# Duankaiwen/LSNet

Measured on AMD Instinct MI355X. Metric: img/s train LSNet R-50-FPN 1333x800 bs2/GPU, higher is better.
Workload: dtype f32 (fp32-equivalent: 6 bf16 MFMA terms per product on exact 3-way operand splits, fp32 accumulate); 1 GPU; LSNet R50-FPN bbox (conv_module_type=dcn), 2 img/GPU 3x800x1344 (1333x800 padded to /32), 7 gt/img, fwd+bwd+gradient arena (the reducer's buckets, no collective on one rank)+clip35+SGD; global_batch=2, parallelism=dp1, world_size=1, memory_format=channels_last, launch=eager

## Files before the change

### lsnet_amd/csrc/conv.hip

```cpp
#include <hip/hip_runtime.h>
#include <stdint.h>
#include <string.h>

#include <type_traits>
#include <vector>

#include "conv_kernels.h"
#include "conv_wgrad_kernels.h"
#include "lib_state.h"
#include "prof.h"

namespace lsn {

static int conv_np() { return math_np() == 0 ? 6 : math_np(); }
static int conv_npl() { return split_npl(conv_np()); }

struct RJob {
    bool fold;
    const float *part, *part_b;
    float *gw, *gb;
    size_t n;
    int nb, splits, splits_b, R, Co;
    WgFold f;
};
// ... 308 lines not shown
struct BwdClass {
    TapSub ts;
    int py, px, pad_h, pad_w, dstep;
    size_t wf_off;
};
struct BwdPlan {
    BwdClass cls[64];
    int ncls;
    bool need_zero;
    size_t bytes;
};

static int bwd_plan(int C, int Co, int kh, int kw, int s, int pad, int dil, BwdPlan *pl)
{
    if (s * s > 64) return fail(LSN_ERR_UNSUPPORTED, "conv2d backward-data: stride %d is not supported", s);
    pl->ncls = 0, pl->need_zero = false, pl->bytes = 0;
    auto taps_of = [&](int p, int k, int &t0, int &tstep, int &nt) {
        t0 = -1, tstep = 1, nt = 0;
        int prev = -1;
        for (int t = 0; t < k; ++t)
            if (((p + pad - t * dil) % s + s) % s == 0) {
                if (nt == 0) t0 = t;
                if (nt == 1) tstep = t - prev;
                prev = t;
                ++nt;
            }
    };
    for (int py = 0; py < s; ++py)
        for (int px = 0; px < s; ++px) {
            BwdClass c;
            c.py = py, c.px = px;
            taps_of(py, kh, c.ts.i0, c.ts.istep, c.ts.ni);
            taps_of(px, kw, c.ts.j0, c.ts.jstep, c.ts.nj);
            c.ts.kw = kw;
            if (c.ts.ni == 0 || c.ts.nj == 0) {
                pl->need_zero = true;
                continue;
            }
            const int dstep_h = c.ts.istep * dil / s, dstep_w = c.ts.jstep * dil / s;
            if (c.ts.ni > 1 && c.ts.nj > 1 && dstep_h != dstep_w)
                return fail(LSN_ERR_UNSUPPORTED, "conv2d backward-data: unequal tap spacing");
            c.dstep = c.ts.ni > 1 ? dstep_h : (c.ts.nj > 1 ? dstep_w : 1);
            if ((c.ts.ni > 1 && c.ts.istep * dil % s != 0) || (c.ts.nj > 1 && c.ts.jstep * dil % s != 0))
                return fail(LSN_ERR_UNSUPPORTED, "conv2d backward-data: stride / dilation combination");
            const int q0h = (py + pad - c.ts.i0 * dil) / s, q0w = (px + pad - c.ts.j0 * dil) / s;
            c.pad_h = (c.ts.ni - 1) * c.dstep - q0h;
            c.pad_w = (c.ts.nj - 1) * c.dstep - q0w;
            c.wf_off = pl->bytes;
            pl->bytes += cv_wfrag_bytes(C, c.ts.ni * c.ts.nj, Co, conv_npl());
            pl->cls[pl->ncls++] = c;
        }
    return 0;
}

static int conv_backward_data_impl(int n, const lsn_conv_level *lv, const void *prepared, int C, int Co, int kh, int kw,
                                   int stride, int pad, int dil, hipStream_t st)
{
    LSN_CHECK(n >= 1 && n <= CV_MAXLV && lv && prepared, "conv2d backward: bad arguments");
    LaunchLog log(1, n, lv, C, C, Co, kh, kw, stride, pad, dil, 0, st);
    if (Co % 4 != 0 && C <= 64) return fail(LSN_ERR_UNSUPPORTED, "conv2d backward-data: Co %% 4 != 0 needs C > 64");
    const int s = stride;
    int Ho[CV_MAXLV], Wo[CV_MAXLV];
    for (int i = 0; i < n; ++i) {
        LSN_CHECK(lv[i].x && lv[i].out, "conv2d backward: NULL tensor in level %d", i);
        if (int rc = conv_check(lv[i].B, lv[i].H, lv[i].W, C, Co, kh, kw, stride, pad, dil, &Ho[i], &Wo[i])) return rc;
    }
    if (s > 1 && n > 1) return fail(LSN_ERR_UNSUPPORTED, "conv2d backward-data: strided convolutions take one level per call");
    BwdPlan pl;
    if (int rc = bwd_plan(C, Co, kh, kw, s, pad, dil, &pl)) return rc;
    const int H = lv[0].H, W = lv[0].W, B = lv[0].B;
    bool epi = false;
    for (int i = 0; i < n; ++i) epi = epi || lv[i].residual || lv[i].gate;
    if (epi && pl.need_zero)
        return fail(LSN_ERR_UNSUPPORTED, "conv2d backward-data: residual / gate with residue classes that have no tap");
    if (epi && C % 4 != 0) return fail(LSN_ERR_UNSUPPORTED, "conv2d backward-data: residual / gate need C %% 4 == 0");
    if (pl.need_zero) LSN_HIP(hipMemsetAsync(lv[0].out, 0, sizeof(float) * (size_t)B * H * W * C, st));
    for (int ci = 0; ci < pl.ncls; ++ci) {
        const BwdClass &c = pl.cls[ci];
        const int Hc = c.py < H ? (H - c.py + s - 1) / s : 0, Wc = c.px < W ? (W - c.px + s - 1) / s : 0;
        if (s > 1 && (Hc == 0 || Wc == 0)) continue;
        ConvArgs a = {};
        a.wf = reinterpret_cast<const unsigned short *>(reinterpret_cast<const unsigned char *>(prepared) + c.wf_off);
        a.wf_bytes = (int)cv_wfrag_bytes(C, c.ts.ni * c.ts.nj, Co, conv_npl());
        a.nlv = n;
        for (int i = 0; i < n; ++i) {
            ConvLvl &L = a.lv[i];
            L.x = lv[i].x, L.out = lv[i].out, L.res = lv[i].residual, L.gate = lv[i].gate;
            L.B = lv[i].B, L.H = Ho[i], L.W = Wo[i];
            L.Ho = s > 1 ? Hc : lv[i].H, L.Wo = s > 1 ? Wc : lv[i].W;
            L.P = L.B * L.Ho * L.Wo;
        }
        a.C = Co, a.Co = C, a.kh = c.ts.ni, a.kw = c.ts.nj, a.stride = 1;
        a.xpitch = Co;
        a.pad_h = c.pad_h, a.pad_w = c.pad_w, a.dil = c.dstep;
        if (s > 1) a.ostep = s, a.oy0 = c.py, a.ox0 = c.px, a.OH = H, a.OW = W;
        ConvProf prof(PROF_CONV_BWD_DATA, a, st);
        if (int rc = conv_forward(a, st)) return rc;
    }
    return 0;
}

static int64_t prepared_bytes(int kind, int C, int Co, int kh, int kw, int stride, int pad, int dil)
{
    if (kind == 0) return (int64_t)cv_wfrag_bytes(Co, kh * kw, C, conv_npl());
    if (kind == 2) return (int64_t)cv_wfrag_bytes(kh * kw * C, 1, Co, conv_npl());
    BwdPlan pl;
    if (bwd_plan(C, Co, kh, kw, stride, pad, dil, &pl)) return -1;
    return (int64_t)pl.bytes;
}

static int bn_fold_of(const lsn_conv_wprep &p, BnFold *bn)
{
    *bn = BnFold();
    if (!p.bn_gamma) return 0;
    LSN_CHECK(p.bn_var, "conv2d prepare: incomplete BatchNorm description");
    if (p.kind == 0)
        LSN_CHECK(p.bn_beta && p.bn_mean && p.shift_out, "conv2d prepare: incomplete BatchNorm description");
    else
        LSN_CHECK(!p.shift_out, "conv2d prepare: the shift belongs to the forward image");
    bn->gamma = p.bn_gamma, bn->var = p.bn_var, bn->beta = p.bn_beta, bn->mean = p.bn_mean, bn->shift_out = p.shift_out;
    bn->eps = p.bn_eps;
    return 0;
}

static int prepare_weights(int kind, const float *w, void *prepared, int C, int Co, int kh, int kw, int stride, int pad,
                           int dil, hipStream_t st, const BnFold &bn = BnFold())
{
    LSN_CHECK(w && prepared, "conv2d prepare: NULL pointer");
    LSN_CHECK(C > 0 && Co > 0 && kh > 0 && kw > 0, "conv2d prepare: bad weight shape");
    if (kh * kw > 64) return fail(LSN_ERR_UNSUPPORTED, "conv2d kernel takes at most 64 taps, got %d x %d", kh, kw);
    if (prepared_bytes(kind, C, Co, kh, kw, stride, pad, dil) >= ((int64_t)1 << 31))
        return fail(LSN_ERR_UNSUPPORTED, "conv2d: weight too large for 32-bit buffer offsets");
    if (kind == 0) {
        if (int rc = conv_wfrag(w, reinterpret_cast<unsigned short *>(prepared), Co, kh * kw, C, 0, TapSub{}, st, bn)) return rc;
    } else if (kind == 2) {
        if (int rc = conv_wfrag(w, reinterpret_cast<unsigned short *>(prepared), kh * kw * C, 1, Co, 1, TapSub{0, 1, 1, 0, 1, 1, 1}, st,
                                bn))
            return rc;
    } else {
        BwdPlan pl;
        if (int rc = bwd_plan(C, Co, kh, kw, stride, pad, dil, &pl)) return rc;
        for (int ci = 0; ci < pl.ncls; ++ci)
            if (int rc = conv_wfrag(w, reinterpret_cast<unsigned short *>(reinterpret_cast<unsigned char *>(prepared) + pl.cls[ci].wf_off),
                                    C, kh * kw, Co, 1, pl.cls[ci].ts, st, bn))
                return rc;
    }
    LSN_HIP(hipGetLastError());
    return 0;
}

static thread_local const WgFoldJobs *g_wg_fold = nullptr;
bool conv_wgrad_fold_pending() { return g_wg_fold != nullptr; }
static int wg_jobs() { return g_wg_fold ? g_wg_fold->njobs : 1; }
template <int TI, int TJ, int TG, int WI, int WJ, int PMAX, bool UN_OK>
static int launch_wgrad_cfg(WgArgs &a, float *gw, float *gb, int accumulate, hipStream_t st)
{
    const bool un = a.Co % 4 != 0;
    if (un && !UN_OK) return 1;
    constexpr int BN = WI * TI * 32, BM = WJ * TJ * 32;
    const int npl = conv_npl(), K = a.kh * a.kw;
    const int blocks = cdiv(a.Co, BM) * cdiv(a.C, BN);
    const size_t nW = (size_t)a.Co * K * a.C;
    const int nj = wg_jobs();
    int S = 512 / (blocks * nj);
    const size_t cap = ((size_t)192 << 20) / 4 / (nW + a.Co) / nj;
    if ((size_t)S > cap) S = (int)cap;
    if (S > a.nseg / nj / 6) S = a.nseg / nj / 6;
    if (S < 1) S = 1;
    S *= nj;
    float *part = nullptr;
    if (int rc = wgrad_part_buffer((size_t)S * (nW + a.Co) + 16, &part, st)) return rc;
    a.part = part;
    a.part_b = part + (((size_t)S * nW + 3) & ~(size_t)3);
    a.want_bias = gb != nullptr;
    constexpr int XP = 1024 / BN, GP = 1024 / BM;
    const size_t lds = (size_t)2 * npl * ((size_t)cdiv(PMAX, XP) * XP * BN * 2 + (size_t)cdiv(16, GP) * GP * BM * 2);
    if (lds > 160 * 1024) return 1;
    dim3 grid(blocks, S);
    LSN_CHECK((long long)a.nseg * (S + 1) < (1ll << 32), "conv2d backward-weight: %d segments x %d splits exceed the kernel's 32-bit split arithmetic", a.nseg, S);
    auto launch = [&](auto kern) -> int {
        LSN_HIP(hipFuncSetAttribute(reinterpret_cast<const void *>(kern), hipFuncAttributeMaxDynamicSharedMemorySize, (int)lds));
        hipLaunchKernelGGL(kern, grid, dim3(256), lds, st, a);
        return 0;
    };
    int rc;
    constexpr bool FINE = !(TG == 9 && WI == 4);
    rc = split_dispatch(conv_np(), [&](auto np) {
        constexpr int NP = decltype(np)::value;
        if constexpr (NP == 1 && TG == 9 && WI == 4) {
            return fail(LSN_ERR_INVALID, "conv2d backward-weight: no one-product form of the narrow 3x3 kernel");
        } else {
            if constexpr (UN_OK) {
                if (un) return launch(conv_wgrad_kernel<TI, TJ, TG, WI, WJ, NP, true, PMAX, false>);
            }
            return launch(conv_wgrad_kernel<TI, TJ, TG, WI, WJ, NP, false, PMAX, FINE>);
        }
    });
    if (rc) return rc;
    return conv_wgrad_reduce(a.part, gw, nW, a.part_b, gb, a.Co, S, S, accumulate, st);
}

static int reduce_ls(int splits)
{
    constexpr int PER_LANE = 16;
    int LS = 1;
    while (LS < 64 && LS * PER_LANE <= splits) LS <<= 1;
    return LS;
}

int conv_wgrad_reduce(const float *part, float *gw, size_t n, const float *part_b, float *gb, int nb, int splits, int splits_b,
                      int accumulate, hipStream_t st)
{
    const int nj = wg_jobs();
    if (g_wg_fold)
        LSN_CHECK(part_b && nb > 0 && n % ((size_t)nb * 4) == 0 && splits % nj == 0 && splits_b % nj == 0,
                  "conv2d backward-weight (folded norm): bad partial layout");
    if (Arena *ar = accumulate ? deferring(st) : nullptr) {
        bool clash = false;
        for (const RJob &q : *ar->jobs)
            for (int j = 0; j < nj; ++j) {
                const float *tw = g_wg_fold ? (nj > 1 ? g_wg_fold->gw[j] : gw) : gw;
                clash = clash || q.gw == tw || (gb && q.gb == gb) || (g_wg_fold && q.fold && q.f.dgamma == g_wg_fold->f[j].dgamma);
            }
        if (clash)
            if (int rc = wgrad_flush(ar)) return rc;
        for (int j = 0; j < nj; ++j) {
            RJob q = {};
            q.fold = g_wg_fold != nullptr;
            q.part = part + (size_t)j * (splits / nj) * n, q.part_b = q.fold ? part_b + (size_t)j * (splits_b / nj) * nb : part_b;
            q.gw = nj > 1 ? g_wg_fold->gw[j] : gw, q.gb = q.fold ? nullptr : gb;
            q.n = n, q.nb = nb, q.splits = splits / nj, q.splits_b = splits_b / nj;
            if (q.fold) q.R = (int)(n / nb), q.Co = nb, q.f = g_wg_fold->f[j];
            ar->jobs->push_back(q);
        }
        if ((long long)(ar->used * sizeof(float)) > (ar->defer_mb << 20)) {
            if (int rc = wgrad_flush(ar)) return rc;
            ar->used = 0;
        }
        return 0;
    }
    const int LS = reduce_ls(splits / nj);
    if (g_wg_fold) {
        hipLaunchKernelGGL(conv_wgrad_reduce_bn_kernel, dim3(nb, nj), dim3(256), 0, st, part, gw, (int)(n / nb), nb, part_b,
                           splits / nj, splits_b / nj, accumulate, LS, *g_wg_fold);
        LSN_HIP(hipGetLastError());
        return 0;
    }
    const size_t thr = n / 4 * LS;
    const int rb = (int)((thr + 255) / 256 < 4096 ? (thr + 255) / 256 : 4096);
    hipLaunchKernelGGL(conv_wgrad_reduce_kernel, dim3(rb > 0 ? rb : 1), dim3(256), 0, st, part, gw, n, part_b, gb, nb, splits,
                       splits_b, accumulate, LS);
    LSN_HIP(hipGetLastError());
    return 0;
}

static int wgrad_flush(Arena *ar)
{
    std::vector<RJob> &jobs = *ar->jobs;
    if (jobs.empty()) return 0;
    hipStream_t st = ar->st;
    double bytes = 0;
    for (const RJob &q : jobs) bytes += 4.0 * ((double)q.splits * q.n + 2.0 * q.n);
    ProfSpan prof(PROF_CONV_WGRAD, 0.0, bytes, st);
    RJobsPlain P = {};
    RJobsFold F = {};
    int pblk = 0, fblk = 0;
    auto launch_plain = [&]() {
        if (P.njobs) hipLaunchKernelGGL(conv_wgrad_reduce_multi_kernel, dim3(pblk), dim3(256), 0, st, P);
        P.njobs = 0, pblk = 0;
    };
    auto launch_fold = [&]() {
        if (F.njobs) hipLaunchKernelGGL(conv_wgrad_reduce_bn_multi_kernel, dim3(fblk), dim3(256), 0, st, F);
        F.njobs = 0, fblk = 0;
    };
    for (const RJob &q : jobs) {
        const int LS = reduce_ls(q.splits);
        if (q.fold) {
            if (F.njobs == RJ_MAX) launch_fold();
            RJobFold &d = F.j[F.njobs++];
            d.part = q.part, d.part_b = q.part_b, d.gw = q.gw, d.f = q.f, d.R = q.R, d.Co = q.Co, d.splits = q.splits,
            d.splits_b = q.splits_b, d.LS = LS, d.blk0 = fblk;
            fblk += q.Co;
        } else {
            if (P.njobs == RJ_MAX) launch_plain();
            const size_t thr = q.n / 4 * LS;
            const int rb = (int)((thr + 255) / 256 < 4096 ? (thr + 255) / 256 : 4096);
            RJobPlain &d = P.j[P.njobs++];
            d.part = q.part, d.part_b = q.part_b, d.gw = q.gw, d.gb = q.gb, d.n = q.n, d.nb = q.nb, d.splits = q.splits,
            d.splits_b = q.splits_b, d.LS = LS, d.blk0 = pblk, d.nblk = rb > 0 ? rb : 1;
            pblk += d.nblk;
        }
    }
    launch_plain();
    launch_fold();
    jobs.clear();
    LSN_HIP(hipGetLastError());
    return 0;
}

int conv_wgrad_mm(int n, const lsn_conv_level *lv, float *gw, float *gb, int C, int Co, int kh, int kw, int stride, int pad,
                  int dil, int accumulate, hipStream_t st)
{
    const bool k33 = kh == 3 && kw == 3 && stride == 1 && dil == 1, k11 = kh == 1 && kw == 1;
    if (n < 1 || n > CV_MAXLV || !(k33 || k11) || C % 4 != 0) return 1;
    WgArgs a = {};
    int seg = 0;
    for (int i = 0; i < n; ++i) {
        WgLvl &L = a.lv[i];
        const int B = lv[i].B, H = lv[i].H, W = lv[i].W;
        if (!lv[i].x || !lv[i].grad_out || B <= 0 || H <= 0 || W <= 0) return 1;
        const int Ho = conv_out_size(H, kh, stride, pad, dil), Wo = conv_out_size(W, kw, stride, pad, dil);
        if (Ho <= 0 || Wo <= 0) return 1;
        if ((int64_t)B * H * W * C * 4 >= ((int64_t)1 << 31) || (int64_t)B * Ho * Wo * Co * 4 >= ((int64_t)1 << 31)) return 1;
        L.x = lv[i].x, L.go = lv[i].grad_out, L.B = B, L.H = H, L.W = W, L.Ho = Ho, L.Wo = Wo;
        L.nsx = cdiv(Wo, 16);
        L.seg0 = seg;
        seg += B * Ho * L.nsx;
    }
    a.nlv = n, a.nseg = seg;
    a.C = C, a.Co = Co, a.kh = kh, a.kw = kw, a.stride = stride, a.pad = pad, a.dil = dil;
    a.cstep = kw == 1 ? stride : 1;
    a.PW = kw == 1 ? 16 : 15 * stride + (kw - 1) * dil + 1;
    if (kh * a.PW > 99) return 1;
    if (kh * kw == 9 && Co <= 32 && conv_np() == 1) return 1;
    double px = 0, in_el = 0;
    for (int i = 0; i < n; ++i) px += (double)a.lv[i].B * a.lv[i].Ho * a.lv[i].Wo, in_el += (double)a.lv[i].B * a.lv[i].H * a.lv[i].W * C;
    ProfSpan prof(PROF_CONV_WGRAD, 2.0 * px * Co * C * kh * kw, 4.0 * (in_el + px * Co + (double)Co * kh * kw * C), st);
    if (kh * kw == 1) {
        if (C <= 64)
            return Co <= 64 ? launch_wgrad_cfg<1, 1, 1, 2, 2, 16, false>(a, gw, gb, accumulate, st)
                            : launch_wgrad_cfg<1, 2, 1, 2, 2, 16, false>(a, gw, gb, accumulate, st);
        return Co <= 64 ? launch_wgrad_cfg<2, 1, 1, 2, 2, 16, false>(a, gw, gb, accumulate, st)
                        : launch_wgrad_cfg<2, 2, 1, 2, 2, 16, false>(a, gw, gb, accumulate, st);
    }
    if (Co <= 32) return launch_wgrad_cfg<1, 1, 9, 4, 1, 54, true>(a, gw, gb, accumulate, st);
    return launch_wgrad_cfg<1, 1, 9, 2, 2, 54, false>(a, gw, gb, accumulate, st);
}

static WfragJob *g_jobs_dev = nullptr;
static size_t g_jobs_cap = 0;
static std::vector<WfragJob> g_jobs_host;

static int prepare_weights_multi(int n, const lsn_conv_wprep *it, hipStream_t st)
{
    LSN_CHECK(n >= 0 && (n == 0 || it), "conv2d prepare: bad item list");
    std::vector<WfragJob> jobs;
    long long total = 0;
    for (int i = 0; i < n; ++i) {
        const lsn_conv_wprep &p = it[i];
        LSN_CHECK(p.w && p.prepared && p.C > 0 && p.Co > 0 && p.kh > 0 && p.kw > 0 && p.kh * p.kw <= 64,
                  "conv2d prepare: bad item %d", i);
        if (prepared_bytes(p.kind, p.C, p.Co, p.kh, p.kw, p.stride, p.pad, p.dil) >= ((int64_t)1 << 31))
            return fail(LSN_ERR_UNSUPPORTED, "conv2d: weight too large for 32-bit buffer offsets");
        BnFold bn;
        if (int rc = bn_fold_of(p, &bn)) return rc;
        auto add = [&](void *out, int Co, int K, int C, int flipT, const TapSub &ts) {
            WfragJob j;
            wfrag_job(j, p.w, reinterpret_cast<unsigned short *>(out), Co, K, C, flipT, ts, bn);
            j.start = total;
            total += wfrag_threads(j);
            jobs.push_back(j);
        };
        if (p.kind == 0) {
            add(p.prepared, p.Co, p.kh * p.kw, p.C, 0, TapSub{});
        } else if (p.kind == 2) {
            add(p.prepared, p.kh * p.kw * p.C, 1, p.Co, 1, TapSub{0, 1, 1, 0, 1, 1, 1});
        } else {
            BwdPlan pl;
            if (int rc = bwd_plan(p.C, p.Co, p.kh, p.kw, p.stride, p.pad, p.dil, &pl)) return rc;
            for (int c = 0; c < pl.ncls; ++c)
                add(reinterpret_cast<unsigned char *>(p.prepared) + pl.cls[c].wf_off, p.C, p.kh * p.kw, p.Co, 1, pl.cls[c].ts);
        }
    }
    if (jobs.empty()) return 0;
    const size_t bytes = jobs.size() * sizeof(WfragJob);
    const bool same = jobs.size() == g_jobs_host.size() && memcmp(jobs.data(), g_jobs_host.data(), bytes) == 0;
    if (!same) {
        if (jobs.size() > g_jobs_cap) {
            LSN_HIP(hipMalloc(reinterpret_cast<void **>(&g_jobs_dev), (jobs.size() + 64) * sizeof(WfragJob)));
            lib_stat(STAT_MALLOCS, 1), lib_stat(STAT_HELD_BYTES, (long long)((jobs.size() + 64) * sizeof(WfragJob)));
            g_jobs_cap = jobs.size() + 64;
        }
        LSN_HIP(hipStreamSynchronize(st));
        lib_stat(STAT_BLOCKING_SYNCS, 1);
        LSN_HIP(hipMemcpy(g_jobs_dev, jobs.data(), bytes, hipMemcpyHostToDevice));
        g_jobs_host = jobs;
    }
    const int blocks = (int)((total + 255) / 256 < 4096 ? (total + 255) / 256 : 4096);
    if (int rc = split_dispatch(conv_np(), [&](auto np) {
            hipLaunchKernelGGL(conv_wfrag_multi_kernel<SplitCfg<decltype(np)::value>::NPL>, dim3(blocks), dim3(256), 0, st, g_jobs_dev,
                               (int)jobs.size(), total);
            return 0;
        }))
        return rc;
    LSN_HIP(hipGetLastError());
    return 0;
}

}

extern "C" {

int lsn_wgrad_defer(int max_mbytes, lsn_stream_t stream)
{
    hipStream_t st = reinterpret_cast<hipStream_t>(stream);
    lsn::Arena *ar = lsn::arena_of(st);
    if (max_mbytes > 0) {
        if (int rc = lsn::arena_get(st, &ar)) return rc;
        if (!ar->jobs) ar->jobs = new std::vector<lsn::RJob>();
        ar->jobs->clear();
        ar->used = 0;
        ar->defer_mb = max_mbytes;
        return 0;
    }
    if (!ar) return 0;
    const int rc = lsn::wgrad_flush(ar);
    ar->defer_mb = 0, ar->used = 0;
    return rc;
}

int lsn_wgrad_flush(lsn_stream_t stream)
{
    lsn::Arena *ar = lsn::arena_of(reinterpret_cast<hipStream_t>(stream));
    if (!ar) return 0;
    const int rc = lsn::wgrad_flush(ar);
    ar->used = 0;
    return rc;
}

int lsn_conv2d_backward_weight_bn(const float *x, const float *g, const float *w, const float *bn_gamma, const float *bn_mean,
                                  const float *bn_var, float bn_eps, float *grad_w, float *grad_gamma, float *grad_beta, int B,
                                  int H, int W, int C, int Co, int kh, int kw, int stride, int pad, int dil, int accumulate,
                                  lsn_stream_t stream)
{
    LSN_CHECK(x && g && w && bn_gamma && bn_mean && bn_var && grad_w && grad_gamma && grad_beta,
              "conv2d backward-weight (folded norm): NULL pointer");
    if (((size_t)kh * kw * C) % 4 != 0)
        return lsn::fail(LSN_ERR_UNSUPPORTED, "conv2d backward-weight (folded norm): kh * kw * C %% 4 != 0");
    lsn::WgFoldJobs f = {};
    f.f[0] = lsn::WgFold{w, bn_gamma, bn_mean, bn_var, grad_gamma, grad_beta, bn_eps};
    f.gw[0] = grad_w, f.njobs = 1;
    lsn::g_wg_fold = &f;
    const int rc = lsn_conv2d_backward_weight(x, g, grad_w, grad_beta, B, H, W, C, Co, kh, kw, stride, pad, dil, accumulate, stream);
    lsn::g_wg_fold = nullptr;
    return rc;
}

int lsn_conv2d_backward_weight_bn_jobs(int n_jobs, const lsn_wgrad_bn_job *jobs, int B, int H, int W, int C, int Co, int kh, int kw,
                                       int stride, int pad, int dil, int accumulate, lsn_stream_t stream)
{
    LSN_CHECK(n_jobs >= 1 && n_jobs <= 8 && jobs, "conv2d backward-weight jobs: 1 .. 8 jobs");
    lsn::WgFoldJobs f = {};
    lsn_conv_level lv[8] = {};
    for (int j = 0; j < n_jobs; ++j) {
        const lsn_wgrad_bn_job &q = jobs[j];
        LSN_CHECK(q.x && q.g && q.w && q.bn_gamma && q.bn_mean && q.bn_var && q.grad_w && q.grad_gamma && q.grad_beta,
                  "conv2d backward-weight jobs: NULL pointer in job %d", j);
        f.f[j] = lsn::WgFold{q.w, q.bn_gamma, q.bn_mean, q.bn_var, q.grad_gamma, q.grad_beta, q.bn_eps};
        f.gw[j] = q.grad_w;
        lv[j].x = q.x, lv[j].grad_out = q.g, lv[j].B = B, lv[j].H = H, lv[j].W = W;
    }
    f.njobs = n_jobs;
    int rc = 1;
    if (n_jobs > 1 && ((size_t)kh * kw * C) % 4 == 0) {
        lsn::g_wg_fold = &f;
        rc = lsn::conv_wgrad_mm(n_jobs, lv, jobs[0].grad_w, jobs[0].grad_beta, C, Co, kh, kw, stride, pad, dil, accumulate,
                                reinterpret_cast<hipStream_t>(stream));
        lsn::g_wg_fold = nullptr;
    }
    if (rc != 1) return rc;
    for (int j = 0; j < n_jobs; ++j) {
        const lsn_wgrad_bn_job &q = jobs[j];
        if (int r = lsn_conv2d_backward_weight_bn(q.x, q.g, q.w, q.bn_gamma, q.bn_mean, q.bn_var, q.bn_eps, q.grad_w, q.grad_gamma,
                                                  q.grad_beta, B, H, W, C, Co, kh, kw, stride, pad, dil, accumulate, stream))
            return r;
    }
    return 0;
}

int lsn_conv2d_prepare_weights_multi(int n_items, const lsn_conv_wprep *items, lsn_stream_t stream)
// ... 96 lines not shown
```

### lsnet_amd/csrc/conv_wgrad_kernels.h

```cpp
#pragma once
#include <hip/hip_runtime.h>
#include <stdint.h>

#include "common.h"
#include "conv_kernels.h"

namespace lsn {

struct WgLvl {
    const float *x, *go;
    int B, H, W, Ho, Wo;
    int nsx;
    int seg0;
};

struct WgArgs {
    WgLvl lv[CV_MAXLV];
    int nlv, nseg;
    int C, Co, kh, kw, stride, pad, dil;
    int PW;
    int cstep;
    float *part;
    float *part_b;
    int want_bias;
// ... 150 lines not shown
        for (int i = 0; i < TI; ++i)
#pragma unroll
            for (int h = 0; h < 2; ++h) {
                const int m = 8 * (lane >> 5) + 4 * h + rb;
                const int pp = (tp / KW) * a.PW + (m * a.stride + (tp % KW) * a.dil) / a.cstep;
                const int sl = (2 * (wi * TI + i) + g) ^ (2 * ((pp >> (RBX == 128 ? 1 : 0)) & (RBX / 64 - 1)));
                xaddr[tp][i][h] = pp * RBX + sl * 32 + cq * 8;
            }
    int gaddr[TJ][2];
#pragma unroll
    for (int j = 0; j < TJ; ++j)
#pragma unroll
        for (int h = 0; h < 2; ++h) {
            const int m = 8 * (lane >> 5) + 4 * h + rb;
            const int sl = (2 * (wj * TJ + j) + g) ^ (2 * ((m >> (RBG == 128 ? 1 : 0)) & (RBG / 64 - 1)));
            gaddr[j][h] = m * RBG + sl * 32 + cq * 8;
        }

    f32x16 acc[TG][TI][TJ];
#pragma unroll
    for (int tp = 0; tp < TG; ++tp)
#pragma unroll
        for (int i = 0; i < TI; ++i)
#pragma unroll
            for (int j = 0; j < TJ; ++j)
#pragma unroll
                for (int r = 0; r < 16; ++r) acc[tp][i][j][r] = 0.f;

    auto frag = [&](const unsigned char *p0, const unsigned char *p1) {
        const s16x4 lo = lds_tr16(p0), hi = lds_tr16(p1);
        typedef unsigned u32x2 __attribute__((ext_vector_type(2)));
        typedef unsigned u32x4 __attribute__((ext_vector_type(4)));
        const u32x2 a2 = __builtin_bit_cast(u32x2, lo), b2 = __builtin_bit_cast(u32x2, hi);
        const u32x4 r = {a2.x, a2.y, b2.x, b2.y};
        return __builtin_bit_cast(bf16x8, r);
    };

    open_seg(s_begin, T > 0);
#pragma unroll
    for (int sl = 0; sl < NSL; ++sl) issue_slice(sl);
#pragma unroll
    for (int sl = 0; sl < NSL; ++sl) commit_slice(sl, smem);
    next_seg(T > 1);
#pragma unroll
    for (int sl = 0; sl < NSL; ++sl) issue_slice(sl);
    __syncthreads();

    for (int t = 0; t < T; ++t) {
        const unsigned char *bc = smem + (t & 1) * STAGE;
        unsigned char *bn = smem + ((t & 1) ^ 1) * STAGE;
        bf16x8 Gf[TJ][NPL], Xf[2][TI][NPL];
#pragma unroll
        for (int j = 0; j < TJ; ++j)
#pragma unroll
            for (int q = 0; q < NPL; ++q)
                Gf[j][q] = frag(bc + NPL * XPL + q * GPL + gaddr[j][0], bc + NPL * XPL + q * GPL + gaddr[j][1]);
#pragma unroll
        for (int i = 0; i < TI; ++i)
#pragma unroll
            for (int q = 0; q < NPL; ++q) Xf[0][i][q] = frag(bc + q * XPL + xaddr[0][i][0], bc + q * XPL + xaddr[0][i][1]);
        next_seg(t + 2 < T);
        __builtin_amdgcn_sched_barrier(0);
        if constexpr (FINE && TG == 1) {
            constexpr int NMt = NP * TI * TJ;
#pragma unroll
            for (int sl = 0; sl < NSL; ++sl) {
#pragma unroll
                for (int m = sl * NMt / NSL; m < (sl + 1) * NMt / NSL; ++m) {
                    const int prod = m / (TI * TJ), i = (m / TJ) % TI, j = m % TJ;
                    acc[0][i][j] = mfma_bf16(Xf[0][i][SC::pa(prod)], Gf[j][SC::pb(prod)], acc[0][i][j]);
                }
                commit_slice(sl, bn);
                issue_slice(sl);
#pragma unroll
                for (int g = 0; g < NMt / NSL; ++g) {
                    __builtin_amdgcn_sched_group_barrier(0x008, 1, 0);
                    __builtin_amdgcn_sched_group_barrier(0x006, 4, 0);
                }
                __builtin_amdgcn_sched_barrier(0);
            }
        } else
#pragma unroll
        for (int tp = 0; tp < TG; ++tp) {
            if (tp + 1 < TG) {
#pragma unroll
                for (int i = 0; i < TI; ++i)
#pragma unroll
                    for (int q = 0; q < NPL; ++q)
                        Xf[(tp + 1) & 1][i][q] = frag(bc + q * XPL + xaddr[tp + 1][i][0], bc + q * XPL + xaddr[tp + 1][i][1]);
            }
#pragma unroll
            for (int prod = 0; prod < NP; ++prod)
#pragma unroll
                for (int i = 0; i < TI; ++i)
#pragma unroll
                    for (int j = 0; j < TJ; ++j)
                        acc[tp][i][j] = mfma_bf16(Xf[tp & 1][i][SC::pa(prod)], Gf[j][SC::pb(prod)], acc[tp][i][j]);
#pragma unroll
            for (int sl = (TG == 1 ? 0 : tp); sl < (TG == 1 ? NSL : (tp < NSL ? tp + 1 : 0)); ++sl) {
                if (FINE || t + 1 < T) commit_slice(sl, bn);
                issue_slice(sl);
            }
            if (TG == 9 && tp == TG - 1) {
#pragma unroll
                for (int sl = TG; sl < NSL; ++sl) {
                    if (FINE || t + 1 < T) commit_slice(sl, bn);
                    issue_slice(sl);
                }
            }
            if constexpr (FINE) {
#pragma unroll
                for (int g = 0; g < NP * TI * TJ; ++g) {
                    __builtin_amdgcn_sched_group_barrier(0x008, 1, 0);
                    __builtin_amdgcn_sched_group_barrier(0x006, 4, 0);
                }
            }
            __builtin_amdgcn_sched_barrier(0);
        }
        __syncthreads();
    }

    const size_t nW = (size_t)a.Co * TG * a.C;
    float *pw = a.part + (size_t)split * nW;
    const bool v4 = (a.C & 3) == 0;
#pragma unroll
    for (int tp = 0; tp < TG; ++tp) {
#pragma unroll
        for (int j = 0; j < TJ; ++j) {
            const int co = co_blk + (wj * TJ + j) * 32 + (lane & 31);
            if (co >= a.Co) continue;
#pragma unroll
            for (int i = 0; i < TI; ++i)
#pragma unroll
                for (int q = 0; q < 4; ++q) {
                    const int ci = ci_blk + (wi * TI + i) * 32 + 8 * q + 4 * (lane >> 5);
                    if (ci >= a.C) continue;
                    float *dst = pw + ((size_t)co * TG + tp) * a.C + ci;
                    if (v4) {
                        *reinterpret_cast<float4 *>(dst) = make_float4(acc[tp][i][j][4 * q], acc[tp][i][j][4 * q + 1],
                                                                       acc[tp][i][j][4 * q + 2], acc[tp][i][j][4 * q + 3]);
                    } else {
#pragma unroll
                        for (int e = 0; e < 4; ++e)
                            if (ci + e < a.C) dst[e] = acc[tp][i][j][4 * q + e];
                    }
                }
        }
    }
    if (do_bias) {
        __syncthreads();
        float *red = reinterpret_cast<float *>(smem);
#pragma unroll
        for (int e = 0; e < 4; ++e) red[(tid / GT) * BM + 4 * gc4 + e] = bacc[e];
        __syncthreads();
        if (tid < BM && co_blk + tid < a.Co) {
            float s = 0.f;
            for (int r = 0; r < GP; ++r) s += red[r * BM + tid];
            a.part_b[(size_t)split * a.Co + co_blk + tid] = s;
        }
    }
}

__device__ __forceinline__ void wgrad_reduce_body(const float *__restrict__ part, float *__restrict__ gw, size_t n,
                                                  const float *__restrict__ part_b, float *__restrict__ gb, int nb, int splits,
                                                  int splits_b, int accumulate, int LS, unsigned vblock, unsigned vgrid)
{
    const size_t n4 = n / 4;
    const size_t gid = vblock * (size_t)blockDim.x + threadIdx.x;
    const size_t stride = (size_t)vgrid * blockDim.x / LS;
    const int sl = (int)(gid % LS);
    for (size_t e0 = gid / LS; e0 < ((n4 + stride - 1) / stride) * stride; e0 += stride) {
        const bool live = e0 < n4;
        const size_t e = live ? e0 : 0;
        float4 s = make_float4(0.f, 0.f, 0.f, 0.f);
        int z = sl;
        for (; z + 3 * LS < splits; z += 4 * LS) {
            const float4 p0 = reinterpret_cast<const float4 *>(part + (size_t)z * n)[e];
            const float4 p1 = reinterpret_cast<const float4 *>(part + (size_t)(z + LS) * n)[e];
            const float4 p2 = reinterpret_cast<const float4 *>(part + (size_t)(z + 2 * LS) * n)[e];
            const float4 p3 = reinterpret_cast<const float4 *>(part + (size_t)(z + 3 * LS) * n)[e];
            s.x += p0.x, s.y += p0.y, s.z += p0.z, s.w += p0.w;
            s.x += p1.x, s.y += p1.y, s.z += p1.z, s.w += p1.w;
            s.x += p2.x, s.y += p2.y, s.z += p2.z, s.w += p2.w;
            s.x += p3.x, s.y += p3.y, s.z += p3.z, s.w += p3.w;
        }
        for (; z < splits; z += LS) {
            const float4 p = reinterpret_cast<const float4 *>(part + (size_t)z * n)[e];
            s.x += p.x, s.y += p.y, s.z += p.z, s.w += p.w;
        }
        for (int m = 1; m < LS; m <<= 1) {
            s.x += __shfl_xor(s.x, m), s.y += __shfl_xor(s.y, m), s.z += __shfl_xor(s.z, m), s.w += __shfl_xor(s.w, m);
        }
        if (live && sl == 0) {
            float4 *d = reinterpret_cast<float4 *>(gw) + e;
            if (accumulate) {
                const float4 o = *d;
                s.x += o.x, s.y += o.y, s.z += o.z, s.w += o.w;
            }
            *d = s;
        }
    }
    if (gb && vblock == 0)
        for (int e = threadIdx.x; e < nb; e += blockDim.x) {
            float s0 = 0.f, s1 = 0.f, s2 = 0.f, s3 = 0.f;
            int z = 0;
            for (; z + 3 < splits_b; z += 4) {
                s0 += part_b[(size_t)z * nb + e], s1 += part_b[(size_t)(z + 1) * nb + e];
                s2 += part_b[(size_t)(z + 2) * nb + e], s3 += part_b[(size_t)(z + 3) * nb + e];
            }
            for (; z < splits_b; ++z) s0 += part_b[(size_t)z * nb + e];
            const float s = (s0 + s1) + (s2 + s3);
            gb[e] = accumulate ? gb[e] + s : s;
        }
}

static __global__ void conv_wgrad_reduce_kernel(const float *__restrict__ part, float *__restrict__ gw, size_t n,
                                                const float *__restrict__ part_b, float *__restrict__ gb, int nb, int splits,
                                                int splits_b, int accumulate, int LS)
{
    wgrad_reduce_body(part, gw, n, part_b, gb, nb, splits, splits_b, accumulate, LS, blockIdx.x, gridDim.x);
}

struct WgFold {
    const float *w, *gamma, *mean, *var;
    float *dgamma, *dbeta;
    float eps;
};
struct WgFoldJobs {
    WgFold f[8];
    float *gw[8];
    int njobs;
};

__device__ __forceinline__ void wgrad_reduce_bn_body(const float *__restrict__ part, float *gw, int R, int Co,
                                                     const float *__restrict__ part_b, int splits, int splits_b, int accumulate,
                                                     int LS, const WgFold &f, int co)
{
    __shared__ float red[2][4];
    const int tid = threadIdx.x, lane = tid & 63, wave = tid >> 6;
    const size_t n = (size_t)Co * R;
    const int sl = tid % LS, el = tid / LS, EP = 256 / LS;
    const float rstd = rsqrtf(f.var[co] + f.eps), ac = f.gamma[co] * rstd;
    const int R4 = R / 4;
    float dot = 0.f;
    for (int e0 = 0; e0 < R4; e0 += EP) {
        const bool live = e0 + el < R4;
        const size_t e = (size_t)co * R4 + (live ? e0 + el : 0);
        float4 s = make_float4(0.f, 0.f, 0.f, 0.f);
        int z = sl;
        for (; z + 3 * LS < splits; z += 4 * LS) {
            const float4 p0 = reinterpret_cast<const float4 *>(part + (size_t)z * n)[e];
            const float4 p1 = reinterpret_cast<const float4 *>(part + (size_t)(z + LS) * n)[e];
            const float4 p2 = reinterpret_cast<const float4 *>(part + (size_t)(z + 2 * LS) * n)[e];
            const float4 p3 = reinterpret_cast<const float4 *>(part + (size_t)(z + 3 * LS) * n)[e];
            s.x += p0.x, s.y += p0.y, s.z += p0.z, s.w += p0.w;
            s.x += p1.x, s.y += p1.y, s.z += p1.z, s.w += p1.w;
            s.x += p2.x, s.y += p2.y, s.z += p2.z, s.w += p2.w;
            s.x += p3.x, s.y += p3.y, s.z += p3.z, s.w += p3.w;
        }
        for (; z < splits; z += LS) {
            const float4 p = reinterpret_cast<const float4 *>(part + (size_t)z * n)[e];
            s.x += p.x, s.y += p.y, s.z += p.z, s.w += p.w;
        }
        for (int m = 1; m < LS; m <<= 1) {
            s.x += __shfl_xor(s.x, m), s.y += __shfl_xor(s.y, m), s.z += __shfl_xor(s.z, m), s.w += __shfl_xor(s.w, m);
        }
        if (live && sl == 0) {
            const float4 wv = reinterpret_cast<const float4 *>(f.w)[e];
            dot += (wv.x * s.x + wv.y * s.y) + (wv.z * s.z + wv.w * s.w);
            float4 *d = reinterpret_cast<float4 *>(gw) + e;
            float4 o;
            if (accumulate) {
                const float4 q = *d;
                o = make_float4(__builtin_fmaf(ac, s.x, q.x), __builtin_fmaf(ac, s.y, q.y), __builtin_fmaf(ac, s.z, q.z),
                                __builtin_fmaf(ac, s.w, q.w));
            } else {
                o = make_float4(ac * s.x, ac * s.y, ac * s.z, ac * s.w);
            }
            *d = o;
        }
    }
    float sb = 0.f;
    for (int z = tid; z < splits_b; z += 256) sb += part_b[(size_t)z * Co + co];
    for (int m = 1; m < 64; m <<= 1) dot += __shfl_xor(dot, m), sb += __shfl_xor(sb, m);
    if (lane == 0) red[0][wave] = dot, red[1][wave] = sb;
    __syncthreads();
    if (tid == 0) {
        const float d4 = (red[0][0] + red[0][1]) + (red[0][2] + red[0][3]);
        const float b4 = (red[1][0] + red[1][1]) + (red[1][2] + red[1][3]);
        const float t = d4 - f.mean[co] * b4;
        f.dbeta[co] = accumulate ? f.dbeta[co] + b4 : b4;
        f.dgamma[co] = accumulate ? __builtin_fmaf(t, rstd, f.dgamma[co]) : t * rstd;
    }
}

static __global__ __launch_bounds__(256) void conv_wgrad_reduce_bn_kernel(const float *__restrict__ part, float *gw, int R, int Co,
                                                                           const float *__restrict__ part_b, int splits,
                                                                           int splits_b, int accumulate, int LS,
                                                                           const WgFoldJobs J)
{
    gw = J.njobs > 1 ? J.gw[blockIdx.y] : gw;
    part += (size_t)blockIdx.y * splits * ((size_t)Co * R);
    part_b += (size_t)blockIdx.y * splits_b * Co;
    wgrad_reduce_bn_body(part, gw, R, Co, part_b, splits, splits_b, accumulate, LS, J.f[blockIdx.y], blockIdx.x);
}

// ... 38 lines not shown
```

Baseline: 68.74 img/s.

## Add specialized 1x1 stride-1 unpadded weight-gradient conv kernel

```diff
diff --git a/lsnet_amd/csrc/conv.hip b/lsnet_amd/csrc/conv.hip
--- a/lsnet_amd/csrc/conv.hip
+++ b/lsnet_amd/csrc/conv.hip
@@ -484,7 +484,7 @@
 static thread_local const WgFoldJobs *g_wg_fold = nullptr;
 bool conv_wgrad_fold_pending() { return g_wg_fold != nullptr; }
 static int wg_jobs() { return g_wg_fold ? g_wg_fold->njobs : 1; }
-template <int TI, int TJ, int TG, int WI, int WJ, int PMAX, bool UN_OK>
+template <int TI, int TJ, int TG, int WI, int WJ, int PMAX, bool UN_OK, bool PLAIN11 = false>
 static int launch_wgrad_cfg(WgArgs &a, float *gw, float *gb, int accumulate, hipStream_t st)
 {
     const bool un = a.Co % 4 != 0;
@@ -519,7 +519,9 @@
     constexpr bool FINE = !(TG == 9 && WI == 4);
     rc = split_dispatch(conv_np(), [&](auto np) {
         constexpr int NP = decltype(np)::value;
-        if constexpr (NP == 1 && TG == 9 && WI == 4) {
+        if constexpr (PLAIN11) {
+            return launch(conv_wgrad_1x1_kernel<TI, TJ, WI, WJ, NP>);
+        } else if constexpr (NP == 1 && TG == 9 && WI == 4) {
             return fail(LSN_ERR_INVALID, "conv2d backward-weight: no one-product form of the narrow 3x3 kernel");
         } else {
             if constexpr (UN_OK) {
@@ -658,6 +660,13 @@
     double px = 0, in_el = 0;
     for (int i = 0; i < n; ++i) px += (double)a.lv[i].B * a.lv[i].Ho * a.lv[i].Wo, in_el += (double)a.lv[i].B * a.lv[i].H * a.lv[i].W * C;
     ProfSpan prof(PROF_CONV_WGRAD, 2.0 * px * Co * C * kh * kw, 4.0 * (in_el + px * Co + (double)Co * kh * kw * C), st);
+    if (kh * kw == 1 && stride == 1 && pad == 0) {
+        if (C <= 64)
+            return Co <= 64 ? launch_wgrad_cfg<1, 1, 1, 2, 2, 16, false, true>(a, gw, gb, accumulate, st)
+                            : launch_wgrad_cfg<1, 2, 1, 2, 2, 16, false, true>(a, gw, gb, accumulate, st);
+        return Co <= 64 ? launch_wgrad_cfg<2, 1, 1, 2, 2, 16, false, true>(a, gw, gb, accumulate, st)
+                        : launch_wgrad_cfg<2, 2, 1, 2, 2, 16, false, true>(a, gw, gb, accumulate, st);
+    }
     if (kh * kw == 1) {
         if (C <= 64)
             return Co <= 64 ? launch_wgrad_cfg<1, 1, 1, 2, 2, 16, false>(a, gw, gb, accumulate, st)
diff --git a/lsnet_amd/csrc/conv_wgrad_kernels.h b/lsnet_amd/csrc/conv_wgrad_kernels.h
--- a/lsnet_amd/csrc/conv_wgrad_kernels.h
+++ b/lsnet_amd/csrc/conv_wgrad_kernels.h
@@ -326,6 +326,232 @@
         float *red = reinterpret_cast<float *>(smem);
 #pragma unroll
         for (int e = 0; e < 4; ++e) red[(tid / GT) * BM + 4 * gc4 + e] = bacc[e];
+        __syncthreads();
+        if (tid < BM && co_blk + tid < a.Co) {
+            float s = 0.f;
+            for (int r = 0; r < GP; ++r) s += red[r * BM + tid];
+            a.part_b[(size_t)split * a.Co + co_blk + tid] = s;
+        }
+    }
+}
+
+template <int TI, int TJ, int WI, int WJ, int NP>
+__global__ __launch_bounds__(256, 2) void conv_wgrad_1x1_kernel(const WgArgs a)
+{
+    using SC = SplitCfg<NP>;
+    constexpr int NPL = SC::NPL;
+    static_assert(WI * WJ == 4, "four waves");
+    constexpr int KP = 16, KG = 1;
+    constexpr int BN = WI * TI * 32, BM = WJ * TJ * 32;
+    constexpr int RBX = BN * 2, RBG = BM * 2;
+    constexpr int XT = BN / 4, XP = 256 / XT, XL = KP / XP;
+    constexpr int GT = BM / 4, GP = 256 / GT, GL = KP / GP;
+    static_assert(KP % XP == 0 && KP % GP == 0, "whole staging passes");
+    constexpr int XPL = KP * RBX, GPL = KP * RBG, STAGE = NPL * (XPL + GPL);
+    constexpr int NSL = XL + GL;
+    constexpr int OOB = 0x7ffffff0;
+    extern __shared__ __align__(16) unsigned char smem[];
+
+    const int tid = threadIdx.x, lane = tid & 63, wave = tid >> 6;
+    const int wi = wave / WJ, wj = wave % WJ;
+    const int nib = (a.C + BN - 1) / BN;
+    const int work = xcd_remap(blockIdx.y * gridDim.x + blockIdx.x, gridDim.x * gridDim.y);
+    const int split = work / (int)gridDim.x, blk = work - split * (int)gridDim.x;
+    const int cb = blk / nib, ib = blk - cb * nib;
+    const int ci_blk = ib * BN, co_blk = cb * BM;
+    const int s_begin = (int)((unsigned)a.nseg * (unsigned)split / gridDim.y);
+    const int T = (int)((unsigned)a.nseg * (unsigned)(split + 1) / gridDim.y) - s_begin;
+
+    const int xc4 = tid % XT, xq = tid / XT;
+    const bool xin = ci_blk + 4 * xc4 < a.C;
+    int xoff[XL], xlds[XL];
+#pragma unroll
+    for (int it = 0; it < XL; ++it) {
+        const int q = it * XP + xq;
+        xoff[it] = (q * a.C + ci_blk + 4 * xc4) * 4;
+        const int sl = (xc4 >> 2) ^ (2 * ((q >> (RBX == 128 ? 1 : 0)) & (RBX / 64 - 1)));
+        xlds[it] = q * RBX + sl * 32 + (xc4 & 3) * 8;
+    }
+    const int gc4 = tid % GT, gq = tid / GT;
+    const bool gin = co_blk + 4 * gc4 < a.Co;
+    int goff[GL], glds[GL];
+#pragma unroll
+    for (int it = 0; it < GL; ++it) {
+        const int q = it * GP + gq;
+        goff[it] = (q * a.Co + co_blk + 4 * gc4) * 4;
+        const int sl = (gc4 >> 2) ^ (2 * ((q >> (RBG == 128 ? 1 : 0)) & (RBG / 64 - 1)));
+        glds[it] = q * RBG + sl * 32 + (gc4 & 3) * 8;
+    }
+
+    float4 xv[XL], gv[GL];
+    float bacc[4] = {0.f, 0.f, 0.f, 0.f};
+    const bool do_bias = a.want_bias && ib == 0;
+
+    struct Step {
+        int s, step_next, sx, nsx, W, row0, p0, lim;
+        __amdgpu_buffer_rsrc_t xrs, grs;
+    } sg;
+    auto open_step = [&](int s, bool live) {
+        int li = 0;
+        while (li + 1 < a.nlv && s >= a.lv[li + 1].seg0) ++li;
+        const WgLvl &L = a.lv[li];
+        const int r = s - L.seg0, P = L.B * L.H * L.W;
+        const int rowid = r / L.nsx;
+        sg.sx = r - rowid * L.nsx, sg.nsx = L.nsx, sg.W = L.W;
+        sg.row0 = rowid * L.W;
+        sg.p0 = sg.row0 + sg.sx * KP;
+        sg.lim = live ? sg.W - sg.sx * KP : 0;
+        sg.xrs = __builtin_amdgcn_make_buffer_rsrc(const_cast<float *>(L.x), 0, P * a.C * 4, 0x00020000);
+        sg.grs = __builtin_amdgcn_make_buffer_rsrc(const_cast<float *>(L.go), 0, P * a.Co * 4, 0x00020000);
+        sg.s = s;
+        sg.step_next = li + 1 < a.nlv ? a.lv[li + 1].seg0 : 0x7fffffff;
+    };
+    auto next_step = [&](bool live) {
+        const int s = sg.s + 1;
+        if (s >= sg.step_next) {
+            open_step(s, live);
+            return;
+        }
+        sg.s = s;
+        if (++sg.sx == sg.nsx) sg.sx = 0, sg.row0 += sg.W;
+        sg.p0 = sg.row0 + sg.sx * KP;
+        sg.lim = live ? sg.W - sg.sx * KP : 0;
+    };
+    auto issue_slice = [&](int sl) {
+        if (sl < XL) {
+            const int it = sl;
+            const bool ok = xin && it * XP + xq < sg.lim;
+            xv[it] = cv_load4(sg.xrs, ok ? xoff[it] + sg.p0 * a.C * 4 : OOB, 0);
+        } else {
+            const int it = sl - XL;
+            const bool ok = gin && it * GP + gq < sg.lim;
+            gv[it] = cv_load4(sg.grs, ok ? goff[it] + sg.p0 * a.Co * 4 : OOB, 0);
+        }
+    };
+    auto commit_slice = [&](int sl, unsigned char *buf) {
+        unsigned p0[NPL], p1[NPL];
+        if (sl < XL) {
+            const int it = sl;
+            split_planes<NPL>(xv[it].x, xv[it].y, p0);
+            split_planes<NPL>(xv[it].z, xv[it].w, p1);
+#pragma unroll
+            for (int q = 0; q < NPL; ++q) *reinterpret_cast<uint2 *>(buf + q * XPL + xlds[it]) = make_uint2(p0[q], p1[q]);
+        } else {
+            const int it = sl - XL;
+            const float bm = do_bias ? 1.f : 0.f;
+            bacc[0] += bm * gv[it].x, bacc[1] += bm * gv[it].y, bacc[2] += bm * gv[it].z, bacc[3] += bm * gv[it].w;
+            split_planes<NPL>(gv[it].x, gv[it].y, p0);
+            split_planes<NPL>(gv[it].z, gv[it].w, p1);
+#pragma unroll
+            for (int q = 0; q < NPL; ++q)
+                *reinterpret_cast<uint2 *>(buf + NPL * XPL + q * GPL + glds[it]) = make_uint2(p0[q], p1[q]);
+        }
+    };
+
+    const int g = (lane >> 4) & 1, rb = (lane >> 2) & 3, cq = lane & 3;
+    int xaddr[TI][2], gaddr[TJ][2];
+#pragma unroll
+    for (int h = 0; h < 2; ++h) {
+        const int m = 8 * (lane >> 5) + 4 * h + rb;
+#pragma unroll
+        for (int i = 0; i < TI; ++i) {
+            const int sl = (2 * (wi * TI + i) + g) ^ (2 * ((m >> (RBX == 128 ? 1 : 0)) & (RBX / 64 - 1)));
+            xaddr[i][h] = m * RBX + sl * 32 + cq * 8;
+        }
+#pragma unroll
+        for (int j = 0; j < TJ; ++j) {
+            const int sl = (2 * (wj * TJ + j) + g) ^ (2 * ((m >> (RBG == 128 ? 1 : 0)) & (RBG / 64 - 1)));
+            gaddr[j][h] = m * RBG + sl * 32 + cq * 8;
+        }
+    }
+
+    f32x16 acc[TI][TJ];
+#pragma unroll
+    for (int i = 0; i < TI; ++i)
+#pragma unroll
+        for (int j = 0; j < TJ; ++j)
+#pragma unroll
+            for (int r = 0; r < 16; ++r) acc[i][j][r] = 0.f;
+
+    auto frag = [&](const unsigned char *p0, const unsigned char *p1) {
+        const s16x4 lo = lds_tr16(p0), hi = lds_tr16(p1);
+        typedef unsigned u32x2 __attribute__((ext_vector_type(2)));
+        typedef unsigned u32x4 __attribute__((ext_vector_type(4)));
+        const u32x2 a2 = __builtin_bit_cast(u32x2, lo), b2 = __builtin_bit_cast(u32x2, hi);
+        const u32x4 r = {a2.x, a2.y, b2.x, b2.y};
+        return __builtin_bit_cast(bf16x8, r);
+    };
+
+    open_step(s_begin, T > 0);
+#pragma unroll
+    for (int sl = 0; sl < NSL; ++sl) issue_slice(sl);
+#pragma unroll
+    for (int sl = 0; sl < NSL; ++sl) commit_slice(sl, smem);
+    next_step(T > 1);
+#pragma unroll
+    for (int sl = 0; sl < NSL; ++sl) issue_slice(sl);
+    __syncthreads();
+
+    for (int t = 0; t < T; ++t) {
+        const unsigned char *bc = smem + (t & 1) * STAGE;
+        unsigned char *bn = smem + ((t & 1) ^ 1) * STAGE;
+        bf16x8 Gf[KG][TJ][NPL], Xf[KG][TI][NPL];
+        auto read_group = [&](int kg) {
+            const unsigned char *bx = bc + kg * 16 * RBX, *bg = bc + NPL * XPL + kg * 16 * RBG;
+#pragma unroll
+            for (int j = 0; j < TJ; ++j)
+#pragma unroll
+                for (int q = 0; q < NPL; ++q) Gf[kg][j][q] = frag(bg + q * GPL + gaddr[j][0], bg + q * GPL + gaddr[j][1]);
+#pragma unroll
+            for (int i = 0; i < TI; ++i)
+#pragma unroll
+                for (int q = 0; q < NPL; ++q) Xf[kg][i][q] = frag(bx + q * XPL + xaddr[i][0], bx + q * XPL + xaddr[i][1]);
+        };
+        read_group(0);
+        next_step(t + 2 < T);
+        __builtin_amdgcn_sched_barrier(0);
+        constexpr int NMt = NP * TI * TJ, NM = KG * NMt;
+#pragma unroll
+        for (int sl = 0; sl < NSL; ++sl) {
+#pragma unroll
+            for (int m = sl * NM / NSL; m < (sl + 1) * NM / NSL; ++m) {
+                const int kg = m / NMt, r = m % NMt;
+                const int prod = r / (TI * TJ), i = (r / TJ) % TI, j = r % TJ;
+                acc[i][j] = mfma_bf16(Xf[kg][i][SC::pa(prod)], Gf[kg][j][SC::pb(prod)], acc[i][j]);
+            }
+            commit_slice(sl, bn);
+            issue_slice(sl);
+#pragma unroll
+            for (int gm = sl * NM / NSL; gm < (sl + 1) * NM / NSL; ++gm) {
+                __builtin_amdgcn_sched_group_barrier(0x008, 1, 0);
+                __builtin_amdgcn_sched_group_barrier(0x006, 4, 0);
+            }
+            __builtin_amdgcn_sched_barrier(0);
+        }
+        __syncthreads();
+    }
+
+    const size_t nW = (size_t)a.Co * a.C;
+    float *pw = a.part + (size_t)split * nW;
+#pragma unroll
+    for (int j = 0; j < TJ; ++j) {
+        const int co = co_blk + (wj * TJ + j) * 32 + (lane & 31);
+        if (co >= a.Co) continue;
+#pragma unroll
+        for (int i = 0; i < TI; ++i)
+#pragma unroll
+            for (int q = 0; q < 4; ++q) {
+                const int ci = ci_blk + (wi * TI + i) * 32 + 8 * q + 4 * (lane >> 5);
+                if (ci >= a.C) continue;
+                *reinterpret_cast<float4 *>(pw + (size_t)co * a.C + ci) =
+                    make_float4(acc[i][j][4 * q], acc[i][j][4 * q + 1], acc[i][j][4 * q + 2], acc[i][j][4 * q + 3]);
+            }
+    }
+    if (do_bias) {
+        __syncthreads();
+        float *red = reinterpret_cast<float *>(smem);
+#pragma unroll
+        for (int e = 0; e < 4; ++e) red[gq * BM + 4 * gc4 + e] = bacc[e];
         __syncthreads();
         if (tid < BM && co_blk + tid < a.Co) {
             float s = 0.f;
```

Result: no change. 69.18 img/s (median of 6 runs) (+0.6%).
